# GEOS-ESM/GEOSradiation_GridComp

Hardware: AMD Instinct MI355X
Metric: columns/sec (LW+SW, 72 layers) (higher is better)
Workload: dtype f32; 1 GPU; BASELINE configs[3] (C360 tile / 8 GPUs) per-GPU share: 97200 columns/GPU, 72 layers, RRTMG_LW (140 g-points) + RRTMG_SW (112 g-points), McICA clouds on 60 % of the columns (ih=1), aerosols on, every column lit; schemes=RRTMG_LW (140 g-points) + RRTMG_SW (112 g-points), columns_per_gpu=97200, layers=72, aerosol=True, hip_streams=2

## Files before the change

geosradiation_gridcomp_amd/csrc/geosrad.hip:

```cpp
#include <hip/hip_runtime.h>

#include <cstdio>
#include <cstdlib>
#include <cstring>
#include <map>
#include <string>
#include <tuple>
#include <vector>
#include <thread>
#include <mutex>
#include <condition_variable>
#include <memory>
#include <atomic>
#include <functional>
#include <chrono>

#include <dlfcn.h>
#include <sched.h>
#include <cstddef>
#include <cstdint>
#include "../../include/geosrad.h"
#include "dev_buf.hpp"
#include "lw_device.hpp"
#include "lw_kernels.hpp"
// ... 814 lines not shown
    {
        size_t t = 0;
        for (const DevBuf<> *b : {&d_ws, &d_ws_sw, &d_ws_ch, &d_ws_lwk, &d_ws_so, &d_ws_drvs[0], &d_ws_drvs[1], &d_ws_hb, &d_io, &d_tab, &d_tab_sw, &d_tab_ch})
            t += b->bytes;
        return t;
    }

    size_t ws_layout(int nc, int nlay, LwArgs<R> &w, Carve c) const
    {
        const size_t cl = (size_t)nlay * nc;
        w.sc = c.take<R>(SC_NFIELD * cl);
        w.scidx = c.take<uint32_t>(cl);
        w.pwvcm = c.take<R>(nc);
        w.colcloudy = c.take<uint8_t>(nc);
        w.perm = c.take<int32_t>(nc);
        w.nclear = c.take<int32_t>(1);
        w.laycloudy = c.take<uint8_t>(cl);
        w.alpha = c.take<R>(cl);
        w.rcorr = c.take<R>(cl);
        w.taucmc = c.take<R>(NG_LW * cl);
        const size_t clp = (size_t)nlay * (((size_t)nc + 255) & ~(size_t)255);
        w.s1 = c.take<uint16_t>(NG_LW * clp);
        w.s2 = c.take<uint16_t>(NG_LW * clp);
        w.part = c.take<R>((size_t)6 * NB_LW * (nlay + 1) * nc);
        w.pfcode = c.take<uint32_t>(lw_split_path ? NB_LW * cl : 0);
        w.pffs = c.take<R>(lw_split_path ? NB_LW * cl : 0);
        return c.off;
    }
    int ensure_ws(int nc, int nlay)
    {
        if (d_ws && nc <= ws_ncol && nlay == ws_nlay) return GEOSRAD_OK;
// ... 57 lines not shown
        out.seg = it->second.d_seg; out.nseg = it->second.nseg; out.jsub = it->second.jsub; out.jhalf = it->second.jhalf;
        nseg_out = it->second.nseg;
        return GEOSRAD_OK;
    }

    template <int MODE, typename Args> int rrtmg_front(hipStream_t st, const Args &A, bool radval = false, R *rvsum = nullptr)
    {
        constexpr bool SW = MODE == 2;
        const dim3 blk(256);
        const unsigned gx = grid256(A.ncol);
        const LwDev<R> *dT = d_T;
        const SwDev<R> *dS = SW ? (const SwDev<R> *)d_S : nullptr;
        span_begin(SW ? 6 : 0, st);
        if constexpr (SW) {
            hipLaunchKernelGGL(k_sw_validate<R>, dim3(gx), blk, 0, st, A);
            if (A.iaer == 10) hipLaunchKernelGGL(k_sw_validate_aer<R>, dim3(gx, A.nlay), blk, 0, st, A);
        } else hipLaunchKernelGGL(k_validate_pwv<R>, dim3(gx), blk, 0, st, A, d_T);
        hipLaunchKernelGGL(k_partition, dim3(1), dim3(1024), 0, st, A.ncol, (const uint8_t *)A.colcloudy, A.perm, A.nclear);
        span_end(st);
        span_begin(SW ? 7 : 1, st);
        if constexpr (SW) hipLaunchKernelGGL(k_sw_setcoef<R>, dim3(gx, A.nlay), blk, 0, st, A, dS);
        else hipLaunchKernelGGL(k_setcoef<R>, dim3(gx, A.nlay), blk, 0, st, A, d_T);
        span_end(st);
        span_begin(2, st);
        hipLaunchKernelGGL(k_overlap<R>, dim3(gx, A.nlay), blk, 0, st, A.ncol, A.ld, A.nlay, A.doy, A.zm, A.alat, (const int32_t *)A.perm,
                           (const int32_t *)A.nclear, dT, A.alpha, A.rcorr, A.laycloudy);
        span_end(st);
        McArgs<R> M{};
        M.ncol = A.ncol; M.ld = A.ld; M.nlay = A.nlay; M.nsubcol = SW ? NG_SW : NG_LW; M.doy = A.doy; M.cloudLM = A.cloudLM; M.cloudMH = A.cloudMH;
        M.iceflg = A.iceflg; M.liqflg = A.liqflg;
        for (int k = 0; k < 4; k++) M.so[k] = SW ? 4 - k : 1 + k;
        M.cwp_tiny = (R)1.e-20;
        M.play = A.play; M.ciwp = A.ciwp; M.clwp = A.clwp; M.rei = A.rei; M.rel = A.rel;
        M.alpha = A.alpha; M.rcorr = A.rcorr; M.perm = A.perm; M.nclear = A.nclear; M.cftop = A.colcloudy;
        M.taucmc = A.taucmc; M.laycloudy = A.laycloudy; M.clearCounts = A.clearCounts; M.err = A.err;
        if constexpr (SW) { M.cldf = A.cld; M.ssacmc = A.ssacmc; M.asmcmc = A.asmcmc; M.cotsum = A.cotsum; M.rvsum = rvsum; }
        else M.cldf = A.cldf;
// ... 99 lines not shown
            auto Q = [&](int k) { return colp(out[k], c0); };
            O.uflx = Q(O_UFLX); O.dflx = Q(O_DFLX); O.uflxc = Q(O_UFLXC); O.dflxc = Q(O_DFLXC);
            O.duflx_dTs = Q(O_DUFLX); O.duflxc_dTs = Q(O_DUFLXC);
            O.olrb = (R *)out[O_OLRB]; O.dolrb_dTs = (R *)out[O_DOLRB]; O.col0 = c0;
            if (const int e = lw_sweeps(st, A, O, nrats <= 0)) return e;

            for (int r = 0; r < nrats; r++) {
                static const R *LwArgs<R>::*const GAS[GEOSRAD_RAT_NGAS] = {&LwArgs<R>::h2o, &LwArgs<R>::o3, &LwArgs<R>::co2, &LwArgs<R>::ch4, &LwArgs<R>::n2o,
                                                                           &LwArgs<R>::cfc11, &LwArgs<R>::cfc12, &LwArgs<R>::cfc22};
                static_assert(GEOSRAD_RAT_H2O == 0 && GEOSRAD_RAT_N2O == 4 && GEOSRAD_RAT_HCFC22 == 7 && GEOSRAD_RAT_NGAS == 8, "GAS follows GEOSRAD_RAT_*");
                LwArgs<R> B = A;
                B.*GAS[rats->gas[r]] = zero;
                if (rats->gas[r] == GEOSRAD_RAT_H2O) B.pwvcm = zero;
                B.dbg_taug = nullptr; B.dbg_pfracs = nullptr;
                B.band_mask = LW_RAT_BANDS[rats->gas[r]];
                span_begin(1, st); hipLaunchKernelGGL(k_setcoef<R>, dim3(grid256(nc), nlay), dim3(256), 0, st, B, d_T); span_end(st);
                LwOut<R> OR{};
                const size_t ro = (size_t)r * (nlay + 1) * ncol + c0;
                OR.uflx = (R *)rats->uflx + ro; OR.dflx = (R *)rats->dflx + ro;
                OR.duflx_dTs = rats->duflx_dTs ? (R *)rats->duflx_dTs + ro : nullptr;
                OR.col0 = c0; OR.part_alt = rat_part; OR.alt_mask = B.band_mask;
                if (const int e = lw_sweeps(st, B, OR, false)) return e;
            }
            return GEOSRAD_OK;
        });
    }

    int drv_reserve(int which, size_t need)
    {
        if (d_ws_drvs[which].reserve(need) != hipSuccess) return fail(GEOSRAD_ENOMEM, "hipMalloc of the driver workspace failed");
        return GEOSRAD_OK;
// ... 536 lines not shown
        if (!any) return GEOSRAD_OK;
        for (int k = 0; k < GEOSRAD_SWHB_NIN; k++)
            if (!in[k]) return fail(GEOSRAD_EINVAL, "null input field");
        HbArgs<R> H{};
        H.lm = lm; H.ld = ncol; H.doy = doy; H.lcldmh = lcldmh; H.lcldlm = lcldlm;
        H.grav = (R)(consts ? consts[GEOSRAD_SWHB_C_GRAV] : 9.80665); H.rgas = (R)(consts ? consts[GEOSRAD_SWHB_C_RGAS] : 8314.47 / 28.965);
        H.cwp_tiny = (R)1.e-20;
        const int nc_max = chunk_cols(ncol);
        const char *ab = getenv("GEOSRAD_SWHB_COMPACT");
        const bool compact = ab ? atoi(ab) != 0 : SWHB_COMPACT;
        int32_t *perm, *nclear;
        auto carve = [&](Carve c) {
            const size_t cl = (size_t)lm * nc_max;
            H.alpha = c.take<R>(cl); H.rcorr = c.take<R>(cl);
            H.cf0 = c.take<uint16_t>(nc_max); H.cf1 = c.take<uint16_t>(nc_max); H.cloudy = c.take<uint8_t>(nc_max);
            perm = c.take<int32_t>(compact ? nc_max : 0); nclear = c.take<int32_t>(compact ? 1 : 0);
            H.cnt = c.take<int32_t>((size_t)4 * nc_max);
            return c.off;
        };
        const size_t need = carve(Carve());
        if (d_ws_hb.reserve(need) != hipSuccess)
            return fail(GEOSRAD_ENOMEM, "hipMalloc of the CLD??SWHB workspace failed (" + std::to_string(need >> 20) + " MiB); lower it with geosrad_set_chunk()");
        carve(Carve(d_ws_hb));
        if (compact) { H.perm = perm; H.nclear = nclear; }
        McPlan MP; int nseg = 0;
        if (const int rc = mc_plan(1, HB_NSUB, lm, MP, nseg)) return rc;
        const LwDev<R> *dT = d_T;
        return chunk_walk(ncol, nc_max, [&](int c0, int nc) {
            H.ncol = nc;
            H.fcld = colp(in[GEOSRAD_SWHB_FCLD], c0); H.ple = colp(in[GEOSRAD_SWHB_PLE], c0); H.t = colp(in[GEOSRAD_SWHB_T], c0);
            H.qi = colp(in[GEOSRAD_SWHB_QI], c0); H.ql = colp(in[GEOSRAD_SWHB_QL], c0); H.lats = colp(in[GEOSRAD_SWHB_LATS], c0);
            for (int k = 0; k < GEOSRAD_SWHB_NOUT; k++) H.out[k] = colp(out[k], c0);
            hipLaunchKernelGGL((k_swhb_prep<R>), dim3(grid256(nc)), dim3(256), 0, st, H, dT);
            if (compact) hipLaunchKernelGGL(k_partition, dim3(1), dim3(1024), 0, st, nc, (const uint8_t *)H.cloudy, perm, nclear);
            hipLaunchKernelGGL((k_swhb_count<R>), dim3(xcd_grid(nc, 64, nseg)), dim3(64), 0, st, H, MP, dT);
            hipLaunchKernelGGL((k_swhb_export<R>), dim3(grid256(nc)), dim3(256), 0, st, H);
            return GEOSRAD_OK;
        });
    }

    int lit_index_dev(hipStream_t st, int ncol, const void *zth, int32_t *idx, int32_t *pos, int32_t *nlit_dev, int *nlit_host) override
    {
        HIPCHK(hipSetDevice(device));
        if (ncol <= 0 || !zth || !idx || !pos || !nlit_dev) return fail(GEOSRAD_EINVAL, "lit_index: bad arguments");
        hipLaunchKernelGGL(k_lit_index<R>, dim3(1), dim3(1024), 0, st, ncol, (const R *)zth, idx, pos, nlit_dev);
        HIPCHK(hipGetLastError());
        if (nlit_host) {
            int32_t v = 0;
            HIPCHK(hipMemcpyAsync(&v, nlit_dev, sizeof v, hipMemcpyDeviceToHost, st));
// ... 184 lines not shown
        for (int b = 1; b <= NB_SW; b++)
            if ((T.b[b].absb && T.b[b].absb < T.b[b].absa) || (T.b[b].x1 && T.b[b].x1 < T.b[b].x0) || d_tab_sw.bytes >= ((size_t)1 << 32))
                return fail(GEOSRAD_ETABLE, "internal: RRTMG_SW table staging order");
        HIPCHK(hipMemcpy(d_S, &h_S, sizeof(SwDev<R>), hipMemcpyHostToDevice));
        have_sw = true;
        return GEOSRAD_OK;
    }

    size_t ws_layout_sw(int nc, int nlay, SwArgs<R> &w, R *&rvsum, Carve c, int planes, bool radval) const
    {
        const size_t cl = (size_t)nlay * nc;
        w.sc = c.take<R>(SW_NFIELD * cl);
        w.scidx = c.take<uint32_t>(cl);
        w.colcloudy = c.take<uint8_t>(nc);
        w.perm = c.take<int32_t>(nc);
        w.nclear = c.take<int32_t>(1);
        w.laycloudy = c.take<uint8_t>(cl);
        w.alpha = c.take<R>(cl);
        w.rcorr = c.take<R>(cl);
        w.taucmc = c.take<R>(NG_SW * cl);
        w.ssacmc = c.take<R>(NG_SW * cl);
        w.asmcmc = c.take<R>(NG_SW * cl);
        w.cotsum = c.take<R>((size_t)3 * NG_SW * nc);
        w.cell = c.take<R>((size_t)planes * NG_SW * nlay * (((size_t)nc + 255) & ~(size_t)255));
        const size_t slots = sw_path == 2 ? (size_t)(sw_reform_nslot<R>() > NB_SW ? sw_reform_nslot<R>() : NB_SW) : (size_t)NB_SW;
        w.part = c.take<R>((size_t)4 * slots * (nlay + 1) * nc);
        w.bsfc = c.take<R>((size_t)3 * slots * nc);
        w.cot = c.take<R>((size_t)8 * 6 * nc);
        rvsum = radval ? c.take<R>((size_t)3 * RV_NSUM * RV_NPAR * nc) : nullptr;
        return c.off;
    }
// ... 1399 lines not shown
```

geosradiation_gridcomp_amd/csrc/lw_cols_kernels.hpp:

```cpp
#pragma once
#include "lw_kernels.hpp"

namespace geosrad {

template <bool CLD> struct LwcK { static constexpr int GR = CLD ? 4 : 8, NST = CLD ? 2 : 1, NPL = 3 * NST; };

__host__ __device__ constexpr int lwc_layer_stride(int nlay) { return 4 * (((nlay + 3) / 4) | 1); }
template <bool CLD> __host__ __device__ constexpr size_t lwc_buf_reals(int nlay, int C)
{
    return (size_t)LwcK<CLD>::NPL * LwcK<CLD>::GR * C * lwc_layer_stride(nlay) + (((size_t)LwcK<CLD>::GR * C * (2 + LwcK<CLD>::NST) + 3) & ~(size_t)3);
}
template <typename R, bool CLD> __host__ __device__ constexpr size_t lwc_lds_bytes(int nlay, int C)
{
    return (2 * lwc_buf_reals<CLD>(nlay, C) + (CLD ? (size_t)10 * ((C * nlay + 63) / 64 * 64) : 0)) * sizeof(R);
}
#ifndef LWC_CMAX
#define LWC_CMAX 8
#endif
template <typename R> __host__ __device__ constexpr int lwc_columns_per_block(int nlay)
{
    return sizeof(R) == 4 ? (nlay <= 72 ? LWC_CMAX : (nlay <= 144 ? LWC_CMAX / 2 : LWC_CMAX / 4))
                          : (nlay <= 72 ? LWC_CMAX / 2 : (nlay <= 144 ? LWC_CMAX / 4 : 1));
}
constexpr int LWC_MAXT = 640;
// ... 155 lines not shown

    Prep<R> P;
    R secdiff = 0, ta = 0, blay = 0, dplankup = 0, dplankdn = 0;
    bool laycld = false;
    if (worker && S.act) {
        BAND::template prep<R>(T, A, S.L, P);
        secdiff = (R)1.66;
        if (!(IB == 1 || IB == 4 || IB >= 10)) {
            constexpr double a0[17] = {0, 1.66, 1.55, 1.58, 1.66, 1.54, 1.454, 1.89, 1.33, 1.668, 1.66, 1.66, 1.66, 1.66, 1.66, 1.66, 1.66};
            constexpr double a1[17] = {0, 0.00, 0.25, 0.22, 0.00, 0.13, 0.446, -0.10, 0.40, -0.006, 0.00, 0.00, 0.00, 0.00, 0.00, 0.00, 0.00};
            constexpr double a2[17] = {0, 0.00, -12.0, -11.7, 0.00, -0.72, -0.243, 0.19, -0.062, 0.414, 0.00, 0.00, 0.00, 0.00, 0.00, 0.00, 0.00};
            secdiff = (R)a0[IB] + (R)a1[IB] * gr_exp<R>((R)a2[IB] * A.pwvcm[S.pc]);
            secdiff = secdiff > (R)1.80 ? (R)1.80 : (secdiff < (R)1.50 ? (R)1.50 : secdiff);
        }
        ta = A.tauaer ? ldg(A.tauaer + (size_t)(IB - 1) * nlay * ld, S.L.ab) : (R)0;
        blay = planck_at<R>(T.totplnk, IB, ldg(A.tlay, S.L.ab));
        const R plk_dn = planck_at<R>(T.totplnk, IB, ldg(A.tlev, S.L.ab));
        const R plk_up = planck_at<R>(T.totplnk, IB, ldg(A.tlev + ld, S.L.ab));
        dplankup = plk_up - blay; dplankdn = plk_dn - blay;
        if (CLD) laycld = A.laycloudy[(size_t)S.lay * n + S.pos] != 0;
    }
    const R *const taucmc_b = CLD ? A.taucmc + (size_t)G0 * nlay * n : nullptr;
    constexpr int W = NG >= 4 ? 4 : 2;

#pragma unroll
    for (int r = 0; r < NR; r++) {
        const int I = I0 + r;
        R *const bcur = lds + (size_t)(I & 1) * bufsz;
        R *const bprev = lds + (size_t)((I + 1) & 1) * bufsz;
        if (worker) {
// ... 159 lines not shown
```

geosradiation_gridcomp_amd/csrc/lw_kernels.hpp:

```cpp
#pragma once
#include "lw_device.hpp"
#include <type_traits>

namespace geosrad {

#define GR_DEV __device__ __forceinline__

template <typename R> GR_DEV R gr_exp(R x);
template <> GR_DEV float gr_exp<float>(float x) { return expf(x); }
template <> GR_DEV double gr_exp<double>(double x) { return exp(x); }
template <typename R> GR_DEV R gr_log(R x);
template <> GR_DEV float gr_log<float>(float x) { return logf(x); }
template <> GR_DEV double gr_log<double>(double x) { return log(x); }
template <typename R> GR_DEV R gr_pow(R x, R y);
template <> GR_DEV float gr_pow<float>(float x, float y) { return powf(x, y); }
template <> GR_DEV double gr_pow<double>(double x, double y) { return pow(x, y); }

#ifndef GR_FAST64
#define GR_FAST64 1
#endif
GR_DEV double gr_rcp64(double b)
{
#if GR_FAST64
    double r = __builtin_amdgcn_rcp(b);
// ... 35 lines not shown
{
    return *reinterpret_cast<const T *>(reinterpret_cast<const char *>(base) + byteoff);
}
template <typename T> GR_DEV void stg(T *base, uint32_t byteoff, T v)
{
    *reinterpret_cast<T *>(reinterpret_cast<char *>(base) + byteoff) = v;
}
template <typename T> GR_DEV T ldg_nt(const T *base, uint32_t byteoff)
{
    return __builtin_nontemporal_load(reinterpret_cast<const T *>(reinterpret_cast<const char *>(base) + byteoff));
}
template <typename T> GR_DEV void stg_nt(T *base, uint32_t byteoff, T v)
{
    __builtin_nontemporal_store(v, reinterpret_cast<T *>(reinterpret_cast<char *>(base) + byteoff));
}
typedef float gr_v2f __attribute__((ext_vector_type(2)));
typedef double gr_v2d __attribute__((ext_vector_type(2)));
template <> GR_DEV float2 ldg_nt<float2>(const float2 *base, uint32_t byteoff)
{
    const gr_v2f t = __builtin_nontemporal_load(reinterpret_cast<const gr_v2f *>(reinterpret_cast<const char *>(base) + byteoff));
    float2 r; r.x = t.x; r.y = t.y; return r;
}
template <> GR_DEV double2 ldg_nt<double2>(const double2 *base, uint32_t byteoff)
{
    const gr_v2d t = __builtin_nontemporal_load(reinterpret_cast<const gr_v2d *>(reinterpret_cast<const char *>(base) + byteoff));
    double2 r; r.x = t.x; r.y = t.y; return r;
}
template <> GR_DEV void stg_nt<float2>(float2 *base, uint32_t byteoff, float2 v)
{
    gr_v2f t; t.x = v.x; t.y = v.y;
// ... 2 lines not shown
template <> GR_DEV void stg_nt<double2>(double2 *base, uint32_t byteoff, double2 v)
{
    gr_v2d t; t.x = v.x; t.y = v.y;
    __builtin_nontemporal_store(t, reinterpret_cast<gr_v2d *>(reinterpret_cast<char *>(base) + byteoff));
}

template <typename R>
__global__ void __launch_bounds__(256) k_validate_pwv(LwArgs<R> A, const LwDev<R> *__restrict__ T)
{
    const int col = blockIdx.x * blockDim.x + threadIdx.x;
    if (col >= A.ncol) return;
    const int ld = A.ld, nlay = A.nlay;
    const R amd = (R)28.9660, amw = (R)18.0160;
    const R grav = T->grav, avogad = T->avogad;
    uint32_t err = 0;
    const R *chk[17] = {A.play, A.tlay, A.h2o, A.o3, A.co2, A.ch4, A.n2o, A.o2, A.cfc11, A.cfc12, A.cfc22, A.ccl4,
                        A.cldf, A.ciwp, A.clwp, A.rei, A.rel};
    R amttl = 0, wvttl = 0;
    int cftop = 0;
    R pprev = A.plev[col];
    if (pprev < 0 || A.tlev[col] < 0) err |= 1u << 17;
    for (int lay = 0; lay < nlay; lay++) {
        const size_t i = (size_t)lay * ld + col;
#pragma unroll
        for (int k = 0; k < 17; k++)
            if (chk[k][i] < 0) err |= 1u << k;
        const R pup = A.plev[i + ld];
        if (pup < 0 || A.tlev[i + ld] < 0) err |= 1u << 17;
        if (A.tauaer)
            for (int ib = 0; ib < NB_LW; ib++)
                if (A.tauaer[((size_t)ib * nlay + lay) * ld + col] < 0) err |= 1u << 20;
        const R h2o = A.h2o[i];
        const R amm = ((R)1. - h2o) * amd + h2o * amw;
        const R coldry = (pprev - pup) * (R)1.e3 * avogad / ((R)1.e2 * grav * amm * ((R)1. + h2o));
        const R btemp = h2o * coldry;
        amttl = amttl + coldry + btemp;
        wvttl = wvttl + btemp;
        if (A.cldf[i] > 0) cftop = lay + 1;
        pprev = pup;
    }
    if (A.tsfc[col] < 0) err |= 1u << 18;
    for (int ib = 0; ib < NB_LW; ib++)
        if (A.emis[(size_t)ib * ld + col] < 0) err |= 1u << 19;
    const R wvsh = (amw * wvttl) / (amd * amttl);
    A.pwvcm[col] = wvsh * ((R)1.e3 * A.plev[col]) / ((R)1.e2 * grav);
    const bool cloudy = cftop > 0;
    A.colcloudy[col] = (uint8_t)cftop;
    for (int k = 0; k < 4; k++) A.clearCounts[(size_t)k * ld + col] = cloudy ? 0 : NG_LW;
    {
        bool upper = false, bad = false;
        for (int lay = 0; lay < nlay; lay++) {
            const bool lower = gr_log<R>(A.play[(size_t)lay * ld + col]) > (R)4.56;
            if (lower && upper) bad = true;
            if (!lower) upper = true;
        }
        if (bad) err |= 1u << ERR_PRESSURE_ORDER;
    }
    if (err) atomicOr(A.err, err);
}

static __global__ void __launch_bounds__(1024) k_partition(int ncol, const uint8_t *__restrict__ colcloudy, int32_t *__restrict__ perm,
                                                    int32_t *__restrict__ nclear)
{
    __shared__ int cnt[1024];
    const int t = threadIdx.x;
    const int chunk = (ncol + 1023) / 1024;
    const int b = t * chunk, e = (b + chunk < ncol) ? b + chunk : ncol;
    int c = 0;
    for (int i = b; i < e; i++) c += colcloudy[i] != 0;
    cnt[t] = c;
    __syncthreads();
    for (int d = 1; d < 1024; d <<= 1) {
        const int v = t >= d ? cnt[t - d] : 0;
        __syncthreads();
        cnt[t] += v;
        __syncthreads();
    }
    const int ncloudy = cnt[1023];
    const int ncl = ncol - ncloudy;
    int cbefore = cnt[t] - c;
    for (int i = b; i < e; i++) {
        if (colcloudy[i]) { perm[ncl + cbefore] = i; cbefore++; }
        else perm[i - cbefore] = i;
    }
    if (t == 0) *nclear = ncl;
}

template <typename R>
__global__ void __launch_bounds__(256) k_setcoef(LwArgs<R> A, const LwDev<R> *__restrict__ T)
{
    const int col = blockIdx.x * blockDim.x + threadIdx.x;
    const int lay = blockIdx.y;
    if (col >= A.ncol) return;
    const int ld = A.ld, n = A.ncol, nlay = A.nlay;
    const size_t i = (size_t)lay * ld + A.perm[col];
    const R amd = (R)28.9660, amw = (R)18.0160;
    const R stpfac = (R)296. / (R)1013.;
    const R pavel = A.play[i], tavel = A.tlay[i], h2o = A.h2o[i];
    const R amm = ((R)1. - h2o) * amd + h2o * amw;
    const R coldry = (A.plev[i] - A.plev[i + ld]) * (R)1.e3 * T->avogad / ((R)1.e2 * T->grav * amm * ((R)1. + h2o));
    const R summol = A.co2[i] + A.o3[i] + A.n2o[i] + A.ch4[i] + A.o2[i];
    const R wbroad = coldry * ((R)1. - summol);
    const R wv = h2o * coldry;

    const R plog = gr_log<R>(pavel);
    const int jp = clampi((int)((R)36. - (R)5 * (plog + (R)0.04)), 1, 58);
    const int jp1 = jp + 1;
    const R fp = (R)5. * (T->preflog[jp - 1] - plog);
    const R dt0 = (tavel - T->tref[jp - 1]) / (R)15.;
    const int jt = clampi((int)((R)3. + dt0), 1, 4);
    const R ft = dt0 - (R)(jt - 3);
    const R dt1 = (tavel - T->tref[jp1 - 1]) / (R)15.;
    const int jt1 = clampi((int)((R)3. + dt1), 1, 4);
    const R ft1 = dt1 - (R)(jt1 - 3);
    const R water = wv / coldry;
    const R scalefac = pavel * stpfac / tavel;
// ... 1035 lines not shown
                    atot = cld ? ac : agas; bbutot = cld ? bbut : bbugas; bbd = cld ? bbdtot : bbdgas;
                }
                rad[g] = rad[g] + (bbd - rad[g]) * atot;
                pend1[j] = (PK)(itp); poff[j] = scell; npend = j + 1;
                dsum = dsum + sumfac * rad[g];
                if (CLD) {
                    const R rc = radc[g] + (bbdgas - radc[g]) * agas;
                    radc[g] = diverge ? rc : rad[g];
                    if (wdv) { pend2[j] = (PK)(itg[j]); pmask2 |= 1u << j; }
                    dcsum = dcsum + sumfac * radc[g];
                }
            }
            __builtin_amdgcn_sched_barrier(0);
        }
        }
        PART(0, lay, dsum);
        if (CLD && ccol) PART(1, lay, dcsum);
    }
#pragma unroll
    for (int j = 0; j < W; j++)
        if (j < npend) {
            stg_nt(s1_b, poff[j] * (uint32_t)sizeof(PK), pend1[j]);
            if (CLD && (pmask2 >> j) & 1u) stg_nt(s2_b, poff[j] * (uint32_t)sizeof(PK), pend2[j]);
        }
    PART(0, nlay, 0);
    if (CLD && ccol) PART(1, nlay, 0);

    int wtop = -1;
    if (CLD) {
        for (int l = nlay - 1; l >= 0; l--)
// ... 219 lines not shown
```

geosradiation_gridcomp_amd/csrc/lw_split_kernels.hpp:

```cpp
#pragma once
#include "lw_kernels.hpp"

namespace geosrad {

constexpr int LWS_CHUNKS = 8;
template <typename R, bool CLD> constexpr int lws_block = sizeof(R) == 4 ? (CLD ? 768 : 1024) : 256;

template <int NG> GR_DEV size_t lws_cell(int ncol_pad, int nlay, int g0, uint32_t ucol, int lay)
{
    return (size_t)g0 * nlay * ncol_pad + (((size_t)(ucol >> 8) * nlay + lay) * 256u + (ucol & 255u)) * NG;
}
typedef uint32_t lws_u4 __attribute__((ext_vector_type(4), aligned(4)));
typedef uint32_t lws_u2 __attribute__((ext_vector_type(2), aligned(4)));
template <int NW> GR_DEV void lws_store(uint16_t *p, const uint32_t (&w)[NW])
{
    uint32_t *q = reinterpret_cast<uint32_t *>(p);
#pragma unroll
    for (int k = 0; k + 4 <= NW; k += 4) { lws_u4 v; v.x = w[k]; v.y = w[k + 1]; v.z = w[k + 2]; v.w = w[k + 3]; __builtin_nontemporal_store(v, reinterpret_cast<lws_u4 *>(q + k)); }
    if constexpr (NW % 4 >= 2) { lws_u2 v; v.x = w[NW / 4 * 4]; v.y = w[NW / 4 * 4 + 1]; __builtin_nontemporal_store(v, reinterpret_cast<lws_u2 *>(q + NW / 4 * 4)); }
    if constexpr (NW % 2 == 1) __builtin_nontemporal_store(w[NW - 1], q + NW - 1);
}
template <int NW> GR_DEV void lws_load(const uint16_t *p, uint32_t (&w)[NW])
{
    const uint32_t *q = reinterpret_cast<const uint32_t *>(p);
// ... 20 lines not shown
        constexpr double a0[17] = {0, 1.66, 1.55, 1.58, 1.66, 1.54, 1.454, 1.89, 1.33, 1.668, 1.66, 1.66, 1.66, 1.66, 1.66, 1.66, 1.66};
        constexpr double a1[17] = {0, 0.00, 0.25, 0.22, 0.00, 0.13, 0.446, -0.10, 0.40, -0.006, 0.00, 0.00, 0.00, 0.00, 0.00, 0.00, 0.00};
        constexpr double a2[17] = {0, 0.00, -12.0, -11.7, 0.00, -0.72, -0.243, 0.19, -0.062, 0.414, 0.00, 0.00, 0.00, 0.00, 0.00, 0.00, 0.00};
        secdiff = (R)a0[IB] + (R)a1[IB] * gr_exp<R>((R)a2[IB] * ldg(A.pwvcm, cba));
        secdiff = secdiff > (R)1.80 ? (R)1.80 : (secdiff < (R)1.50 ? (R)1.50 : secdiff);
    }
    const bool ccol = CLD && col >= nclear;
    const int ctop = CLD && ccol ? (int)A.colcloudy[pc] - 1 : -1;
    const uint32_t npad = ((uint32_t)n + 255u) & ~255u;
    const R *const taucmc_b = A.taucmc + (size_t)G0 * nlay * n;
    const size_t selb = (size_t)(IB - 1) * nlay * n + ucol;
    for (int lay = lay0; lay < lay1; lay++) {
        Layer<R> L;
        load_layer<R>(A, lay, col, pc, L);
        const R ta = A.tauaer ? ldg(A.tauaer + (size_t)(IB - 1) * nlay * ld, L.ab) : (R)0;
        const bool laycld = CLD && ccol && A.laycloudy[(size_t)lay * n + ucol] != 0;
        Prep<R> P;
        BAND::template prep<R>(T, A, L, P);
        PfSel<R> sel{0, 1, (R)0};
        uint32_t wt[NW], wg[NW];
#pragma unroll
        for (int k = 0; k < NW; k++) { wt[k] = 0; wg[k] = 0; }
#pragma unroll
        for (int q = 0; q < NQ; q++) {
            R tau[W], pf[W];
            BAND::template eval<R, W>(T, L, P, q * W, tau, pf, &sel);
#pragma unroll
            for (int j = 0; j < W; j++) {
                const int g = q * W + j;
                if (g >= NG) continue;
// ... 269 lines not shown
```

geosradiation_gridcomp_amd/csrc/sw_kernels.hpp:

```cpp
#pragma once
#include "lw_kernels.hpp"

namespace geosrad {

constexpr int NB_SW = 14;
constexpr int NG_SW = 112;

enum SwGas { G_H2O = 0, G_CO2, G_O3, G_CH4, G_O2, G_NONE };
enum SwScField {
    SW_FAC00 = 0, SW_FAC01, SW_FAC10, SW_FAC11, SW_COLH2O, SW_COLCO2, SW_COLO3, SW_COLCH4, SW_COLO2, SW_COLMOL,
    SW_SELFFAC, SW_SELFFRAC, SW_FORFAC, SW_FORFRAC, SW_NFIELD
};

template <typename R> struct SwBandTab {
    const R *absa, *absb, *selfref, *forref;
    const R *sflux, *irrad, *facb, *snsp;
    const R *rayl;
    const R *x0, *x1;
    const R *raylb;
};

template <typename R> struct SwDev {
    SwBandTab<R> b[NB_SW + 1];
    const R *preflog, *tref;
// ... 31 lines not shown
    R *dbg_taug, *dbg_taur, *dbg_ssi;
};

template <typename R> struct SwOut {
    R *swuflx, *swdflx, *swuflxc, *swdflxc, *nirr, *nirf, *parr, *parf, *uvrr, *uvrf, *fswband, *cot[8], *drband, *dfband;
};

enum SwErr { SWERR_PLEV = 12, SWERR_ALB = 13, SWERR_AER = 14 };

template <typename R>
__global__ void __launch_bounds__(256) k_sw_validate(SwArgs<R> A)
{
    const int col = blockIdx.x * blockDim.x + threadIdx.x;
    if (col >= A.ncol) return;
    const int ld = A.ld, nlay = A.nlay;
    uint32_t err = 0;
    const R *chk[12] = {A.play, A.tlay, A.h2o, A.o3, A.co2, A.ch4, A.o2, A.cld, A.ciwp, A.clwp, A.rei, A.rel};
    int cftop = 0;
    for (int lay = 0; lay < nlay; lay++) {
        const size_t i = (size_t)lay * ld + col;
#pragma unroll
        for (int k = 0; k < 12; k++)
            if (chk[k][i] < 0) err |= 1u << k;
        if (A.plev[i] < 0) err |= 1u << SWERR_PLEV;
        if (A.cld[i] > 0) cftop = lay + 1;
    }
    if (A.plev[(size_t)nlay * ld + col] < 0) err |= 1u << SWERR_PLEV;
    if (A.asdir[col] < 0 || A.aldir[col] < 0 || A.asdif[col] < 0 || A.aldif[col] < 0) err |= 1u << SWERR_ALB;
    const bool cloudy = cftop > 0;
    A.colcloudy[col] = (uint8_t)cftop;
    for (int k = 0; k < 4; k++) A.clearCounts[(size_t)k * ld + col] = cloudy ? 0 : NG_SW;
    if (err) atomicOr(A.err, err);
}

template <typename R>
__global__ void __launch_bounds__(256) k_sw_validate_aer(SwArgs<R> A)
{
    const int col = blockIdx.x * blockDim.x + threadIdx.x;
    const int lay = blockIdx.y;
    if (col >= A.ncol) return;
    bool bad = false;
    for (int ib = 0; ib < NB_SW; ib++) {
        const size_t j = ((size_t)ib * A.nlay + lay) * A.ld + col;
        bad |= A.tauaer[j] < 0 || A.ssaaer[j] < 0;
    }
    if (bad) atomicOr(A.err, 1u << SWERR_AER);
}

template <typename R>
__global__ void __launch_bounds__(256) k_sw_setcoef(SwArgs<R> A, const SwDev<R> *__restrict__ T)
{
    const int col = blockIdx.x * blockDim.x + threadIdx.x;
    const int lay = blockIdx.y;
    if (col >= A.ncol) return;
    const int ld = A.ld, n = A.ncol, nlay = A.nlay;
    const size_t i = (size_t)lay * ld + A.perm[col];
    const R amd = (R)28.9660, amw = (R)18.0160, stpfac = (R)296. / (R)1013.;
    const R pavel = A.play[i], tavel = A.tlay[i], h = A.h2o[i];
    const R coldry = (A.plev[i] - A.plev[i + ld]) * (R)1.e3 * T->avogad /
                     ((R)1.e2 * T->grav * (((R)1. - h) * amd + h * amw) * ((R)1. + h));
    R colh2o = coldry * h, colco2 = coldry * A.co2[i], colo3 = coldry * A.o3[i], colch4 = coldry * A.ch4[i], colo2 = coldry * A.o2[i];
    const R plog = gr_log<R>(pavel);
    const int jp = clampi((int)((R)36. - (R)5 * (plog + (R)0.04)), 1, 58);
    const R fp = (R)5. * (T->preflog[jp - 1] - plog);
    const R d0 = (tavel - T->tref[jp - 1]) / (R)15.;
    const int jt = clampi((int)((R)3. + d0), 1, 4);
    const R ft = d0 - (R)(jt - 3);
    const R d1 = (tavel - T->tref[jp]) / (R)15.;
    const int jt1 = clampi((int)((R)3. + d1), 1, 4);
    const R ft1 = d1 - (R)(jt1 - 3);
    const R water = colh2o / coldry;
    const R scalefac = pavel * stpfac / tavel;
    const bool lower = !(plog <= (R)4.56);
    R forfac = scalefac / ((R)1. + water), forfrac, selffac = 0, selffrac = 0;
    int indfor, indself = 1;
    if (!lower) {
// ... 395 lines not shown

    R prup[NG], prupd[NG], prupT[NG], prupdT[NG];
    int lowc[NG];
#pragma unroll
    for (int g = 0; g < NG; g++) { prup[g] = albp; prupd[g] = albd; prupT[g] = albp; prupdT[g] = albd; lowc[g] = 0x7fffffff; }
    for (int lay = 0; lay < nlay; lay++) {
        SwLayer<R> L;
        sw_load_layer<R>(A, lay, col, L);
        SwPrep<R> P;
        sw_prep<R, B>(T, L, P);
        R ta = 0, om = 1, as = 0;
        if (A.iaer == 10) {
            const uint32_t ab = ((uint32_t)lay * (uint32_t)ld + (uint32_t)pc) * (uint32_t)sizeof(R);
            const size_t bo = (size_t)(IBM - 1) * nlay * ld;
            ta = ldg(A.tauaer + bo, ab); om = ldg(A.ssaaer + bo, ab); as = ldg(A.asmaer + bo, ab);
        }
        const uint32_t cell0 = ((uint32_t)lay * (uint32_t)NG) * (uint32_t)n + ucol;
        const bool laycld = CLD && ccol && ldg(A.laycloudy, (uint32_t)lay * (uint32_t)n + ucol) != 0;
        const bool wlc = CLD && __ballot(laycld) != 0;
#pragma unroll
        for (int q = 0; q < NQ; q++) {
            R tcv[W], ocv[W], gcv[W];
#pragma unroll
            for (int j = 0; j < W; j++) { tcv[j] = 0; ocv[j] = 0; gcv[j] = 0; }
            if (wlc) {
#pragma unroll
                for (int j = 0; j < W; j++)
                    if (q * W + j < NG) tcv[j] = ldg(tcb, (cell0 + (uint32_t)(q * W + j) * (uint32_t)n) * (uint32_t)sizeof(R));
            }
            R tg[W], tr[W];
// ... 350 lines not shown
```

geosradiation_gridcomp_amd/csrc/sw_reform_kernels.hpp:

```cpp
#pragma once
#include "sw_kernels.hpp"

namespace geosrad {

template <typename B> struct SwrRaylPerG { static constexpr bool value = B::JB >= 23 && B::JB <= 27; };

#ifndef SWR_U
#define SWR_U 6
#endif
#ifndef SWR_U64
#define SWR_U64 4
#endif
template <typename R> constexpr int swr_u = sizeof(R) == 8 ? SWR_U64 : SWR_U;
__host__ __device__ constexpr int swr_nunit(int U, int ng) { return (ng + U - 1) / U; }
__host__ __device__ constexpr int swr_usize(int U, int ng, int u)
{
    const int nu = swr_nunit(U, ng);
    if (nu == 1) return ng;
    const int pairs = ng / 2, base = pairs / nu, extra = pairs % nu;
    return 2 * (base + (u < extra ? 1 : 0));
}
__host__ __device__ constexpr int swr_ustart(int U, int ng, int u) { int s = 0; for (int k = 0; k < u; k++) s += swr_usize(U, ng, k); return s; }
__host__ __device__ constexpr int swr_slot0(int U, int jb) { int s = 0; for (int b = 16; b < jb; b++) s += swr_nunit(U, sw_band_ng(b)); return s; }
template <typename R> constexpr int swr_nslot = swr_slot0(swr_u<R>, 30);
// ... 166 lines not shown
                            sw_cell_cloud<R>(c, tcv[j], ocv[j], gcv[j], prmu0, rmu0, t);
                            if constexpr (!REFORM) { PST(10, ct4, t.ref); PST(11, ct4, t.refd); PST(12, ct4, t.tra); PST(13, ct4, t.trad); PST(14, ct4, t.dbt); }
                        }
                        const R zrj = f_rcp<R>((R)1. - prupdT[g] * t.refd);
                        const R pu = t.ref + (t.trad * ((t.tra - t.dbt) * prupdT[g] + t.dbt * prupT[g])) * zrj;
                        const R pd = t.refd + t.trad * t.trad * prupdT[g] * zrj;
                        prupT[g] = pu; prupdT[g] = pd;
                        PST(3, ct4, pu); PST(4, ct4, pd);
                    }
                }
            }
#ifndef SWR_NO_GROUP_BARRIER
            __builtin_amdgcn_sched_barrier(0);
#endif
        }
    }

    const size_t qs = (size_t)swr_nslot<R> * (nlay + 1) * n;
    R *const part = A.part + (size_t)SLOT * (nlay + 1) * n;
#ifdef SWR_PART_NT
#define PART(kind, lev, val) stg_nt(part + (size_t)(kind) * qs + (size_t)(lev) * n, cb, (R)(val))
#else
#define PART(kind, lev, val) stg(part + (size_t)(kind) * qs + (size_t)(lev) * n, cb, (R)(val))
#endif
    R tdbt[NG], ztdn[NG], prdnd[NG], tdbtT[NG], ztdnT[NG], prdndT[NG];
    uint32_t dmask = 0;
    {
        R cu = 0, cd = 0, fu = 0, fd = 0;
#pragma unroll
        for (int g = 0; g < NG; g++) {
// ... 332 lines not shown
```

Baseline: 5.249 million columns/s.

## Fold input validation into setcoef/sweeps and parallelize column partition across blocks

Moves the per-column negative-value checks out of the serial validate kernels into the per-(column,layer) setcoef kernels and into the band sweeps (for aerosol checks), so the inputs are read once where they are already loaded. The separate SW aerosol validation kernel is removed. The single-block 1024-thread partition is replaced by a two-pass multi-block count and scatter using wave ballots. The cost is extra atomics and branches inside hot sweep kernels and an extra small count kernel launch.

```diff
diff --git a/geosradiation_gridcomp_amd/csrc/geosrad.hip b/geosradiation_gridcomp_amd/csrc/geosrad.hip
--- a/geosradiation_gridcomp_amd/csrc/geosrad.hip
+++ b/geosradiation_gridcomp_amd/csrc/geosrad.hip
@@ -852,7 +852,7 @@
         w.pwvcm = c.take<R>(nc);
         w.colcloudy = c.take<uint8_t>(nc);
         w.perm = c.take<int32_t>(nc);
-        w.nclear = c.take<int32_t>(1);
+        w.nclear = c.take<int32_t>(1 + part_blocks(nc));
         w.laycloudy = c.take<uint8_t>(cl);
         w.alpha = c.take<R>(cl);
         w.rcorr = c.take<R>(cl);
@@ -940,13 +940,12 @@
         span_begin(SW ? 6 : 0, st);
         if constexpr (SW) {
             hipLaunchKernelGGL(k_sw_validate<R>, dim3(gx), blk, 0, st, A);
-            if (A.iaer == 10) hipLaunchKernelGGL(k_sw_validate_aer<R>, dim3(gx, A.nlay), blk, 0, st, A);
         } else hipLaunchKernelGGL(k_validate_pwv<R>, dim3(gx), blk, 0, st, A, d_T);
-        hipLaunchKernelGGL(k_partition, dim3(1), dim3(1024), 0, st, A.ncol, (const uint8_t *)A.colcloudy, A.perm, A.nclear);
+        launch_partition(st, A.ncol, A.colcloudy, A.perm, A.nclear);
         span_end(st);
         span_begin(SW ? 7 : 1, st);
         if constexpr (SW) hipLaunchKernelGGL(k_sw_setcoef<R>, dim3(gx, A.nlay), blk, 0, st, A, dS);
-        else hipLaunchKernelGGL(k_setcoef<R>, dim3(gx, A.nlay), blk, 0, st, A, d_T);
+        else hipLaunchKernelGGL((k_setcoef<R, true>), dim3(gx, A.nlay), blk, 0, st, A, d_T);
         span_end(st);
         span_begin(2, st);
         hipLaunchKernelGGL(k_overlap<R>, dim3(gx, A.nlay), blk, 0, st, A.ncol, A.ld, A.nlay, A.doy, A.zm, A.alat, (const int32_t *)A.perm,
@@ -1076,7 +1075,7 @@
                 if (rats->gas[r] == GEOSRAD_RAT_H2O) B.pwvcm = zero;
                 B.dbg_taug = nullptr; B.dbg_pfracs = nullptr;
                 B.band_mask = LW_RAT_BANDS[rats->gas[r]];
-                span_begin(1, st); hipLaunchKernelGGL(k_setcoef<R>, dim3(grid256(nc), nlay), dim3(256), 0, st, B, d_T); span_end(st);
+                span_begin(1, st); hipLaunchKernelGGL((k_setcoef<R, false>), dim3(grid256(nc), nlay), dim3(256), 0, st, B, d_T); span_end(st);
                 LwOut<R> OR{};
                 const size_t ro = (size_t)r * (nlay + 1) * ncol + c0;
                 OR.uflx = (R *)rats->uflx + ro; OR.dflx = (R *)rats->dflx + ro;
@@ -1643,7 +1642,7 @@
             const size_t cl = (size_t)lm * nc_max;
             H.alpha = c.take<R>(cl); H.rcorr = c.take<R>(cl);
             H.cf0 = c.take<uint16_t>(nc_max); H.cf1 = c.take<uint16_t>(nc_max); H.cloudy = c.take<uint8_t>(nc_max);
-            perm = c.take<int32_t>(compact ? nc_max : 0); nclear = c.take<int32_t>(compact ? 1 : 0);
+            perm = c.take<int32_t>(compact ? nc_max : 0); nclear = c.take<int32_t>(compact ? 1 + part_blocks(nc_max) : 0);
             H.cnt = c.take<int32_t>((size_t)4 * nc_max);
             return c.off;
         };
@@ -1661,7 +1660,7 @@
             H.qi = colp(in[GEOSRAD_SWHB_QI], c0); H.ql = colp(in[GEOSRAD_SWHB_QL], c0); H.lats = colp(in[GEOSRAD_SWHB_LATS], c0);
             for (int k = 0; k < GEOSRAD_SWHB_NOUT; k++) H.out[k] = colp(out[k], c0);
             hipLaunchKernelGGL((k_swhb_prep<R>), dim3(grid256(nc)), dim3(256), 0, st, H, dT);
-            if (compact) hipLaunchKernelGGL(k_partition, dim3(1), dim3(1024), 0, st, nc, (const uint8_t *)H.cloudy, perm, nclear);
+            if (compact) launch_partition(st, nc, H.cloudy, perm, nclear);
             hipLaunchKernelGGL((k_swhb_count<R>), dim3(xcd_grid(nc, 64, nseg)), dim3(64), 0, st, H, MP, dT);
             hipLaunchKernelGGL((k_swhb_export<R>), dim3(grid256(nc)), dim3(256), 0, st, H);
             return GEOSRAD_OK;
@@ -1876,7 +1875,7 @@
         w.scidx = c.take<uint32_t>(cl);
         w.colcloudy = c.take<uint8_t>(nc);
         w.perm = c.take<int32_t>(nc);
-        w.nclear = c.take<int32_t>(1);
+        w.nclear = c.take<int32_t>(1 + part_blocks(nc));
         w.laycloudy = c.take<uint8_t>(cl);
         w.alpha = c.take<R>(cl);
         w.rcorr = c.take<R>(cl);
diff --git a/geosradiation_gridcomp_amd/csrc/lw_cols_kernels.hpp b/geosradiation_gridcomp_amd/csrc/lw_cols_kernels.hpp
--- a/geosradiation_gridcomp_amd/csrc/lw_cols_kernels.hpp
+++ b/geosradiation_gridcomp_amd/csrc/lw_cols_kernels.hpp
@@ -193,6 +193,7 @@
             secdiff = secdiff > (R)1.80 ? (R)1.80 : (secdiff < (R)1.50 ? (R)1.50 : secdiff);
         }
         ta = A.tauaer ? ldg(A.tauaer + (size_t)(IB - 1) * nlay * ld, S.L.ab) : (R)0;
+        if (ta < 0) atomicOr(A.err, 1u << 20);
         blay = planck_at<R>(T.totplnk, IB, ldg(A.tlay, S.L.ab));
         const R plk_dn = planck_at<R>(T.totplnk, IB, ldg(A.tlev, S.L.ab));
         const R plk_up = planck_at<R>(T.totplnk, IB, ldg(A.tlev + ld, S.L.ab));
diff --git a/geosradiation_gridcomp_amd/csrc/lw_kernels.hpp b/geosradiation_gridcomp_amd/csrc/lw_kernels.hpp
--- a/geosradiation_gridcomp_amd/csrc/lw_kernels.hpp
+++ b/geosradiation_gridcomp_amd/csrc/lw_kernels.hpp
@@ -73,6 +73,12 @@
 {
     __builtin_nontemporal_store(v, reinterpret_cast<T *>(reinterpret_cast<char *>(base) + byteoff));
 }
+GR_DEV void err_wave(bool bad, uint32_t *err, int bit)
+{
+    if (__ballot(bad) != 0) {
+        if (bad) atomicOr(err, 1u << bit);
+    }
+}
 typedef float gr_v2f __attribute__((ext_vector_type(2)));
 typedef double gr_v2d __attribute__((ext_vector_type(2)));
 template <> GR_DEV float2 ldg_nt<float2>(const float2 *base, uint32_t byteoff)
@@ -105,22 +111,14 @@
     const R amd = (R)28.9660, amw = (R)18.0160;
     const R grav = T->grav, avogad = T->avogad;
     uint32_t err = 0;
-    const R *chk[17] = {A.play, A.tlay, A.h2o, A.o3, A.co2, A.ch4, A.n2o, A.o2, A.cfc11, A.cfc12, A.cfc22, A.ccl4,
-                        A.cldf, A.ciwp, A.clwp, A.rei, A.rel};
     R amttl = 0, wvttl = 0;
     int cftop = 0;
     R pprev = A.plev[col];
     if (pprev < 0 || A.tlev[col] < 0) err |= 1u << 17;
+    bool upper = false, bad = false;
     for (int lay = 0; lay < nlay; lay++) {
         const size_t i = (size_t)lay * ld + col;
-#pragma unroll
-        for (int k = 0; k < 17; k++)
-            if (chk[k][i] < 0) err |= 1u << k;
         const R pup = A.plev[i + ld];
-        if (pup < 0 || A.tlev[i + ld] < 0) err |= 1u << 17;
-        if (A.tauaer)
-            for (int ib = 0; ib < NB_LW; ib++)
-                if (A.tauaer[((size_t)ib * nlay + lay) * ld + col] < 0) err |= 1u << 20;
         const R h2o = A.h2o[i];
         const R amm = ((R)1. - h2o) * amd + h2o * amw;
         const R coldry = (pprev - pup) * (R)1.e3 * avogad / ((R)1.e2 * grav * amm * ((R)1. + h2o));
@@ -128,8 +126,12 @@
         amttl = amttl + coldry + btemp;
         wvttl = wvttl + btemp;
         if (A.cldf[i] > 0) cftop = lay + 1;
+        const bool lower = gr_log<R>(A.play[i]) > (R)4.56;
+        if (lower && upper) bad = true;
+        if (!lower) upper = true;
         pprev = pup;
     }
+    if (bad) err |= 1u << ERR_PRESSURE_ORDER;
     if (A.tsfc[col] < 0) err |= 1u << 18;
     for (int ib = 0; ib < NB_LW; ib++)
         if (A.emis[(size_t)ib * ld + col] < 0) err |= 1u << 19;
@@ -138,46 +140,78 @@
     const bool cloudy = cftop > 0;
     A.colcloudy[col] = (uint8_t)cftop;
     for (int k = 0; k < 4; k++) A.clearCounts[(size_t)k * ld + col] = cloudy ? 0 : NG_LW;
-    {
-        bool upper = false, bad = false;
-        for (int lay = 0; lay < nlay; lay++) {
-            const bool lower = gr_log<R>(A.play[(size_t)lay * ld + col]) > (R)4.56;
-            if (lower && upper) bad = true;
-            if (!lower) upper = true;
-        }
-        if (bad) err |= 1u << ERR_PRESSURE_ORDER;
-    }
     if (err) atomicOr(A.err, err);
 }
 
-static __global__ void __launch_bounds__(1024) k_partition(int ncol, const uint8_t *__restrict__ colcloudy, int32_t *__restrict__ perm,
-                                                    int32_t *__restrict__ nclear)
-{
-    __shared__ int cnt[1024];
-    const int t = threadIdx.x;
-    const int chunk = (ncol + 1023) / 1024;
-    const int b = t * chunk, e = (b + chunk < ncol) ? b + chunk : ncol;
+constexpr int PART_TILE = 1024;
+inline int part_blocks(int ncol) { return (ncol + PART_TILE - 1) / PART_TILE; }
+
+static __global__ void __launch_bounds__(256) k_partition_count(int ncol, const uint8_t *__restrict__ colcloudy, int32_t *__restrict__ tilecnt)
+{
+    const int i0 = blockIdx.x * PART_TILE + threadIdx.x;
     int c = 0;
-    for (int i = b; i < e; i++) c += colcloudy[i] != 0;
-    cnt[t] = c;
+    for (int k = 0; k < PART_TILE / 256; k++) {
+        const int i = i0 + k * 256;
+        c += __syncthreads_count(i < ncol && colcloudy[i] != 0);
+    }
+    if (threadIdx.x == 0) tilecnt[blockIdx.x] = c;
+}
+
+static __global__ void __launch_bounds__(256) k_partition(int ncol, const uint8_t *__restrict__ colcloudy, int32_t *__restrict__ perm,
+                                                   int32_t *__restrict__ nclear, const int32_t *__restrict__ tilecnt)
+{
+    constexpr int NK = PART_TILE / 256, NW = 256 / 64;
+    __shared__ int wcnt[NK * NW];
+    __shared__ int sums[2];
+    const int t = threadIdx.x, lane = t & 63, w = t >> 6;
+    const int i0 = blockIdx.x * PART_TILE + t;
+    if (t < 2) sums[t] = 0;
+    bool f[NK];
+    int pre[NK];
+#pragma unroll
+    for (int k = 0; k < NK; k++) {
+        const int i = i0 + k * 256;
+        f[k] = i < ncol && colcloudy[i] != 0;
+        const unsigned long long m = __ballot(f[k]);
+        pre[k] = __popcll(m & ((1ull << lane) - 1ull));
+        if (lane == 0) wcnt[k * NW + w] = __popcll(m);
+    }
     __syncthreads();
-    for (int d = 1; d < 1024; d <<= 1) {
-        const int v = t >= d ? cnt[t - d] : 0;
+    int before = 0, total = 0;
+    if (gridDim.x > 1) {
+        for (int b = t; b < (int)gridDim.x; b += 256) {
+            const int v = tilecnt[b];
+            total += v;
+            if (b < (int)blockIdx.x) before += v;
+        }
+        if (before) atomicAdd(&sums[0], before);
+        if (total) atomicAdd(&sums[1], total);
         __syncthreads();
-        cnt[t] += v;
-        __syncthreads();
-    }
-    const int ncloudy = cnt[1023];
-    const int ncl = ncol - ncloudy;
-    int cbefore = cnt[t] - c;
-    for (int i = b; i < e; i++) {
-        if (colcloudy[i]) { perm[ncl + cbefore] = i; cbefore++; }
-        else perm[i - cbefore] = i;
-    }
-    if (t == 0) *nclear = ncl;
-}
-
-template <typename R>
+        before = sums[0]; total = sums[1];
+    } else {
+        for (int j = 0; j < NK * NW; j++) total += wcnt[j];
+    }
+    const int ncl = ncol - total;
+#pragma unroll
+    for (int k = 0; k < NK; k++) {
+        const int i = i0 + k * 256;
+        if (i >= ncol) continue;
+        int cb = before + pre[k];
+        for (int j = 0; j < k * NW + w; j++) cb += wcnt[j];
+        if (f[k]) perm[ncl + cb] = i;
+        else perm[i - cb] = i;
+    }
+    if (blockIdx.x == 0 && t == 0) *nclear = ncl;
+}
+
+static inline void launch_partition(hipStream_t st, int ncol, const uint8_t *colcloudy, int32_t *perm, int32_t *nclear)
+{
+    const int nb = part_blocks(ncol);
+    if (nb > 1) hipLaunchKernelGGL(k_partition_count, dim3(nb), dim3(256), 0, st, ncol, colcloudy, nclear + 1);
+    hipLaunchKernelGGL(k_partition, dim3(nb), dim3(256), 0, st, ncol, colcloudy, perm, nclear, (const int32_t *)(nclear + 1));
+}
+
+template <typename R, bool CHECK>
 __global__ void __launch_bounds__(256) k_setcoef(LwArgs<R> A, const LwDev<R> *__restrict__ T)
 {
     const int col = blockIdx.x * blockDim.x + threadIdx.x;
@@ -188,9 +222,20 @@
     const R amd = (R)28.9660, amw = (R)18.0160;
     const R stpfac = (R)296. / (R)1013.;
     const R pavel = A.play[i], tavel = A.tlay[i], h2o = A.h2o[i];
+    const R pdn = A.plev[i], pup = A.plev[i + ld], o3 = A.o3[i], co2 = A.co2[i], ch4 = A.ch4[i], n2o = A.n2o[i], o2 = A.o2[i];
+    if constexpr (CHECK) {
+        const R v[17] = {pavel, tavel, h2o, o3, co2, ch4, n2o, o2, A.cfc11[i], A.cfc12[i], A.cfc22[i], A.ccl4[i],
+                         A.cldf[i], A.ciwp[i], A.clwp[i], A.rei[i], A.rel[i]};
+        uint32_t err = 0;
+#pragma unroll
+        for (int k = 0; k < 17; k++)
+            if (v[k] < 0) err |= 1u << k;
+        if (pup < 0 || A.tlev[i + ld] < 0) err |= 1u << 17;
+        if (err) atomicOr(A.err, err);
+    }
     const R amm = ((R)1. - h2o) * amd + h2o * amw;
-    const R coldry = (A.plev[i] - A.plev[i + ld]) * (R)1.e3 * T->avogad / ((R)1.e2 * T->grav * amm * ((R)1. + h2o));
-    const R summol = A.co2[i] + A.o3[i] + A.n2o[i] + A.ch4[i] + A.o2[i];
+    const R coldry = (pdn - pup) * (R)1.e3 * T->avogad / ((R)1.e2 * T->grav * amm * ((R)1. + h2o));
+    const R summol = co2 + o3 + n2o + ch4 + o2;
     const R wbroad = coldry * ((R)1. - summol);
     const R wv = h2o * coldry;
 
@@ -1256,6 +1301,7 @@
             __builtin_amdgcn_sched_barrier(0);
         }
         }
+        err_wave(ta < 0, A.err, 20);
         PART(0, lay, dsum);
         if (CLD && ccol) PART(1, lay, dcsum);
     }
diff --git a/geosradiation_gridcomp_amd/csrc/lw_split_kernels.hpp b/geosradiation_gridcomp_amd/csrc/lw_split_kernels.hpp
--- a/geosradiation_gridcomp_amd/csrc/lw_split_kernels.hpp
+++ b/geosradiation_gridcomp_amd/csrc/lw_split_kernels.hpp
@@ -58,6 +58,7 @@
         Layer<R> L;
         load_layer<R>(A, lay, col, pc, L);
         const R ta = A.tauaer ? ldg(A.tauaer + (size_t)(IB - 1) * nlay * ld, L.ab) : (R)0;
+        err_wave(ta < 0, A.err, 20);
         const bool laycld = CLD && ccol && A.laycloudy[(size_t)lay * n + ucol] != 0;
         Prep<R> P;
         BAND::template prep<R>(T, A, L, P);
diff --git a/geosradiation_gridcomp_amd/csrc/sw_kernels.hpp b/geosradiation_gridcomp_amd/csrc/sw_kernels.hpp
--- a/geosradiation_gridcomp_amd/csrc/sw_kernels.hpp
+++ b/geosradiation_gridcomp_amd/csrc/sw_kernels.hpp
@@ -69,38 +69,16 @@
     const int col = blockIdx.x * blockDim.x + threadIdx.x;
     if (col >= A.ncol) return;
     const int ld = A.ld, nlay = A.nlay;
-    uint32_t err = 0;
-    const R *chk[12] = {A.play, A.tlay, A.h2o, A.o3, A.co2, A.ch4, A.o2, A.cld, A.ciwp, A.clwp, A.rei, A.rel};
     int cftop = 0;
-    for (int lay = 0; lay < nlay; lay++) {
-        const size_t i = (size_t)lay * ld + col;
-#pragma unroll
-        for (int k = 0; k < 12; k++)
-            if (chk[k][i] < 0) err |= 1u << k;
-        if (A.plev[i] < 0) err |= 1u << SWERR_PLEV;
-        if (A.cld[i] > 0) cftop = lay + 1;
-    }
-    if (A.plev[(size_t)nlay * ld + col] < 0) err |= 1u << SWERR_PLEV;
-    if (A.asdir[col] < 0 || A.aldir[col] < 0 || A.asdif[col] < 0 || A.aldif[col] < 0) err |= 1u << SWERR_ALB;
+    for (int lay = 0; lay < nlay; lay++)
+        if (A.cld[(size_t)lay * ld + col] > 0) cftop = lay + 1;
     const bool cloudy = cftop > 0;
     A.colcloudy[col] = (uint8_t)cftop;
     for (int k = 0; k < 4; k++) A.clearCounts[(size_t)k * ld + col] = cloudy ? 0 : NG_SW;
-    if (err) atomicOr(A.err, err);
-}
-
-template <typename R>
-__global__ void __launch_bounds__(256) k_sw_validate_aer(SwArgs<R> A)
-{
-    const int col = blockIdx.x * blockDim.x + threadIdx.x;
-    const int lay = blockIdx.y;
-    if (col >= A.ncol) return;
-    bool bad = false;
-    for (int ib = 0; ib < NB_SW; ib++) {
-        const size_t j = ((size_t)ib * A.nlay + lay) * A.ld + col;
-        bad |= A.tauaer[j] < 0 || A.ssaaer[j] < 0;
-    }
-    if (bad) atomicOr(A.err, 1u << SWERR_AER);
-}
+    if (A.asdir[col] < 0 || A.aldir[col] < 0 || A.asdif[col] < 0 || A.aldif[col] < 0) atomicOr(A.err, 1u << SWERR_ALB);
+}
+
+template <typename R> GR_DEV void sw_assert_aer(const SwArgs<R> &A, R ta, R om) { err_wave(ta < 0 || om < 0, A.err, SWERR_AER); }
 
 template <typename R>
 __global__ void __launch_bounds__(256) k_sw_setcoef(SwArgs<R> A, const SwDev<R> *__restrict__ T)
@@ -112,9 +90,19 @@
     const size_t i = (size_t)lay * ld + A.perm[col];
     const R amd = (R)28.9660, amw = (R)18.0160, stpfac = (R)296. / (R)1013.;
     const R pavel = A.play[i], tavel = A.tlay[i], h = A.h2o[i];
-    const R coldry = (A.plev[i] - A.plev[i + ld]) * (R)1.e3 * T->avogad /
+    const R pdn = A.plev[i], pup = A.plev[i + ld], co2 = A.co2[i], o3 = A.o3[i], ch4 = A.ch4[i], o2 = A.o2[i];
+    {
+        const R v[12] = {pavel, tavel, h, o3, co2, ch4, o2, A.cld[i], A.ciwp[i], A.clwp[i], A.rei[i], A.rel[i]};
+        uint32_t err = 0;
+#pragma unroll
+        for (int k = 0; k < 12; k++)
+            if (v[k] < 0) err |= 1u << k;
+        if (pdn < 0 || pup < 0) err |= 1u << SWERR_PLEV;
+        if (err) atomicOr(A.err, err);
+    }
+    const R coldry = (pdn - pup) * (R)1.e3 * T->avogad /
                      ((R)1.e2 * T->grav * (((R)1. - h) * amd + h * amw) * ((R)1. + h));
-    R colh2o = coldry * h, colco2 = coldry * A.co2[i], colo3 = coldry * A.o3[i], colch4 = coldry * A.ch4[i], colo2 = coldry * A.o2[i];
+    R colh2o = coldry * h, colco2 = coldry * co2, colo3 = coldry * o3, colch4 = coldry * ch4, colo2 = coldry * o2;
     const R plog = gr_log<R>(pavel);
     const int jp = clampi((int)((R)36. - (R)5 * (plog + (R)0.04)), 1, 58);
     const R fp = (R)5. * (T->preflog[jp - 1] - plog);
@@ -540,6 +528,7 @@
             const uint32_t ab = ((uint32_t)lay * (uint32_t)ld + (uint32_t)pc) * (uint32_t)sizeof(R);
             const size_t bo = (size_t)(IBM - 1) * nlay * ld;
             ta = ldg(A.tauaer + bo, ab); om = ldg(A.ssaaer + bo, ab); as = ldg(A.asmaer + bo, ab);
+            sw_assert_aer<R>(A, ta, om);
         }
         const uint32_t cell0 = ((uint32_t)lay * (uint32_t)NG) * (uint32_t)n + ucol;
         const bool laycld = CLD && ccol && ldg(A.laycloudy, (uint32_t)lay * (uint32_t)n + ucol) != 0;
diff --git a/geosradiation_gridcomp_amd/csrc/sw_reform_kernels.hpp b/geosradiation_gridcomp_amd/csrc/sw_reform_kernels.hpp
--- a/geosradiation_gridcomp_amd/csrc/sw_reform_kernels.hpp
+++ b/geosradiation_gridcomp_amd/csrc/sw_reform_kernels.hpp
@@ -204,6 +204,7 @@
             __builtin_amdgcn_sched_barrier(0);
 #endif
         }
+        sw_assert_aer<R>(A, ta, om);
     }
 
     const size_t qs = (size_t)swr_nslot<R> * (nlay + 1) * n;
```

Result: faster. 5.325 million columns/s (median of 6 runs) (+1.5%).
